# batra-mlp-lab/visdial

Hardware: NVIDIA H100
Metric: QA-rounds/sec mn-att-ques-im-hist+disc train step (higher is better)
Workload: dtype f16 operands + f16 saved state for the option LSTM, tf32 operands elsewhere; fp32 accumulate, fp32 cell state / gradients / optimiser

## Files before the change

visdial_b200/csrc/lstm16.cu:

```cuda
#include <cuda.h>
#include <cuda_fp16.h>
#include <map>
#include <mutex>
#include "../../include/visdial_b200.h"
#include "kernels.cuh"
#include "tc_ptx.cuh"

namespace vd {
namespace tc {

constexpr int BM16 = 128;
constexpr int BK16 = 64;
constexpr int UK16 = 16;
constexpr int BN16 = 128;
constexpr int EW16 = 8;
constexpr int STAGE16 = 32768;

__device__ __forceinline__ float tanh16(float x) { float y; asm("tanh.approx.f32 %0, %1;" : "=f"(y) : "f"(x)); return y; }
__device__ __forceinline__ float sig16(float x) { return fmaf(0.5f, tanh16(0.5f * x), 0.5f); }

__device__ __forceinline__ uint32_t pack2(float a, float b) {
  uint32_t r;
  asm("{\n .reg .f16 lo, hi;\n cvt.rn.satfinite.f16.f32 lo, %1;\n cvt.rn.satfinite.f16.f32 hi, %2;\n mov.b32 %0, {lo, hi};\n}"
      : "=r"(r) : "f"(a), "f"(b));
// ... 10 lines not shown

constexpr int T16_BYTES = 1024, T32_BYTES = 2048;
__device__ __forceinline__ uint8_t* t16_at(uint8_t* base, int row, int unit) {
  return base + row * 64 + (((unit >> 3) ^ ((row >> 1) & 3)) << 4) + (unit & 7) * 2;
}
__device__ __forceinline__ uint8_t* t32_at(uint8_t* base, int row, int unit) {
  return base + row * 128 + (((unit >> 2) ^ (row & 7)) << 4) + (unit & 3) * 4;
}
__device__ __forceinline__ const void* shfl_vptr(const void* p, int src_lane) {
  unsigned long long v = (unsigned long long)p;
  unsigned lo = __shfl_sync(0xffffffffu, (unsigned)v, src_lane), hi = __shfl_sync(0xffffffffu, (unsigned)(v >> 32), src_lane);
  return (const void*)(((unsigned long long)hi << 32) | lo);
}
__device__ __forceinline__ void cp16(void* dst, const void* src) {
  asm volatile("cp.async.cg.shared.global [%0], [%1], 16;" ::"r"(smem_u32(dst)), "l"(src) : "memory");
}
__device__ __forceinline__ void t16_load(uint8_t* base, const void* mine, int lane) {
#pragma unroll
  for (int ps = 0; ps < 2; ++ps) {
    const int row = ps * 8 + (lane >> 2), c = lane & 3;
    const uint8_t* src = (const uint8_t*)shfl_vptr(mine, row);
    uint8_t* dst = base + row * 64 + ((c ^ ((row >> 1) & 3)) << 4);
    if (src) cp16(dst, src + c * 16); else *reinterpret_cast<uint4*>(dst) = make_uint4(0, 0, 0, 0);
  }
}
__device__ __forceinline__ void t32_load(uint8_t* base, const void* mine, int lane) {
#pragma unroll
  for (int ps = 0; ps < 4; ++ps) {
    const int row = ps * 4 + (lane >> 3), c = lane & 7;
    const uint8_t* src = (const uint8_t*)shfl_vptr(mine, row);
    uint8_t* dst = base + row * 128 + ((c ^ (row & 7)) << 4);
    if (src) cp16(dst, src + c * 16); else *reinterpret_cast<float4*>(dst) = make_float4(0.f, 0.f, 0.f, 0.f);
  }
}
__device__ __forceinline__ void cp_wait_all() {
  asm volatile("cp.async.wait_all;" ::: "memory");
  __syncwarp();
}
__device__ __forceinline__ float2 ld_h2(uint8_t* p) { return __half22float2(*reinterpret_cast<const __half2*>(p)); }
__device__ __forceinline__ void st_h2(uint8_t* p, float a, float b) { *reinterpret_cast<uint32_t*>(p) = pack2(a, b); }

struct Lstm16Params {
  int R, H;
  const __half* ptable; const int32_t* tok;
  const float* bias;
  const float* c_prev;
  const int32_t* mask_ids;
  float* h32_out;
  int save_gates;
  const __half* gsave; const float* c_cur; float* dc_carry;
};
struct Lstm16Maps { CUtensorMap g16, c, h16; };

template <int MODE>
struct Cfg16 {
  static constexpr int THREADS = 128 + 32 * EW16;
  static constexpr int STG_PER_WARP = MODE == 0 ? (5 * T16_BYTES + T32_BYTES) : (4 * T16_BYTES + 3 * T32_BYTES);
  static constexpr int STG_BYTES = EW16 * STG_PER_WARP;
  static constexpr int STAGES = (232448 - 1024 - 256 - STG_BYTES) / STAGE16;
  static constexpr int TOTAL = STAGES * STAGE16 + STG_BYTES + 1024 + 256;
};

template <int MODE>
__global__ void __launch_bounds__(Cfg16<MODE>::THREADS, 1)
k_lstm16(const __grid_constant__ CUtensorMap tmA, const __grid_constant__ CUtensorMap tmB,
         const __grid_constant__ Lstm16Maps em, const Lstm16Params p) {
  using C = Cfg16<MODE>;
  constexpr int STAGES = C::STAGES;
  extern __shared__ uint8_t smem_raw[];
  uint8_t* smem = (uint8_t*)(((uintptr_t)smem_raw + 1023) & ~(uintptr_t)1023);
  uint8_t* stg_all = smem + STAGES * STAGE16;
  uint64_t* full = (uint64_t*)(stg_all + C::STG_BYTES);
  uint64_t* empty = full + STAGES;

  const int warp = threadIdx.x >> 5, lane = threadIdx.x & 31;
  const int H = p.H;
  const int num_m = (p.R + BM16 - 1) / BM16;
  const int num_n = MODE == 0 ? H / 32 : H / BN16;
  const int num_tiles = num_m * num_n;
  const int num_kb = (MODE == 0 ? H : 4 * H) / BK16;

  if (threadIdx.x == 0) {
    for (int s = 0; s < STAGES; ++s) { mbar_init(&full[s], 1); mbar_init(&empty[s], 2); }
    asm volatile("fence.mbarrier_init.release.cluster;" ::: "memory");
  }
  __syncthreads();

  if (warp < 4) {
    if (threadIdx.x == 0) {
      int s = 0; uint32_t ph = 0;
      for (int tile = blockIdx.x; tile < num_tiles; tile += gridDim.x) {
        const int m0 = (tile / num_n) * BM16;
        const int nt = tile % num_n;
        for (int kb = 0; kb < num_kb; ++kb) {
          mbar_wait(&empty[s], ph ^ 1);
          uint8_t* sa = smem + s * STAGE16;
          uint8_t* sb = sa + 16384;
          mbar_expect_tx(&full[s], STAGE16);
          tma_load_2d(sa, &tmA, &full[s], kb * BK16, m0);
          if (MODE == 0) {
#pragma unroll
            for (int g = 0; g < 4; ++g) tma_load_2d(sb + g * 4096, &tmB, &full[s], kb * BK16, g * H + nt * 32);
          } else {
            tma_load_2d(sb, &tmB, &full[s], kb * BK16, nt * BN16);
          }
          if (++s == STAGES) { s = 0; ph ^= 1; }
        }
      }
    }
  } else {
    const int cw = warp - 4, wg = cw >> 2;
    uint8_t* stg = stg_all + cw * C::STG_PER_WARP;
    const int fr = lane >> 2, fu = 2 * (lane & 3);
    int s = 0; uint32_t ph = 0;
    auto contract = [&](float (&d)[BN16 / 2]) {
#pragma unroll
      for (int i = 0; i < BN16 / 2; ++i) d[i] = 0.f;
      int prev = -1;
      for (int kb = 0; kb < num_kb; ++kb) {
        mbar_wait(&full[s], ph);
        const uint32_t sa = smem_u32(smem + s * STAGE16);
        const uint64_t adesc = make_desc(sa + wg * 64 * 128, 16, 1024), bdesc = make_desc(sa + 16384, 16, 1024);
        wgmma_fence();
#pragma unroll
        for (int k = 0; k < BK16 / UK16; ++k)
          wgmma_f16_n128(d, adesc + (uint64_t)(k * 2), bdesc + (uint64_t)(k * 2), (kb | k) ? 1u : 0u);
        wgmma_commit();
        wgmma_wait<1>();
        if (prev >= 0 && (threadIdx.x & 127) == 0) mbar_arrive(&empty[prev]);
        prev = s;
        if (++s == STAGES) { s = 0; ph ^= 1; }
      }
      wgmma_wait<0>();
      wgmma_hold(d);
      if (prev >= 0 && (threadIdx.x & 127) == 0) mbar_arrive(&empty[prev]);
    };
    if constexpr (MODE == 0) {
      uint8_t* sG = stg; uint8_t* sH = stg + 4 * T16_BYTES; uint8_t* sC = sH + T16_BYTES;
      for (int tile = blockIdx.x; tile < num_tiles; tile += gridDim.x) {
        const int m0 = (tile / num_n) * BM16;
        const int nt = tile % num_n;
        const int r0 = m0 + wg * 64 + (cw & 3) * 16;
        const int j0 = nt * 32;
        const int64_t row = (int64_t)r0 + (lane & 15);
        const bool row_ok = row < p.R;
        const float keep = (row_ok && p.mask_ids && p.mask_ids[row] == 0) ? 0.f : 1.f;
        const int32_t tk = row_ok ? __ldg(p.tok + row) : 0;
        const __half* prow = tk != 0 ? p.ptable + (int64_t)tk * 4 * H + j0 : nullptr;
        const float* cprow = (row_ok && p.c_prev) ? p.c_prev + row * H + j0 : nullptr;
        if (lane == 0) bulk_wait_read0();
        __syncwarp();
#pragma unroll
        for (int g = 0; g < 4; ++g) t16_load(sG + g * T16_BYTES, prow ? prow + g * H : nullptr, lane);
        t32_load(sC, cprow, lane);
        float d[BN16 / 2];
        contract(d);
        cp_wait_all();
#pragma unroll
        for (int hh = 0; hh < 2; ++hh) {
          const int r = fr + 8 * hh;
          const float kp = __shfl_sync(0xffffffffu, keep, r);
          const int64_t grow = (int64_t)r0 + r;
#pragma unroll
          for (int jj = 0; jj < 4; ++jj) {
            const int u = 8 * jj + fu;
            float a[4][2], cp[2], hn[2];
#pragma unroll
            for (int g = 0; g < 4; ++g) {
              const float2 x = ld_h2(t16_at(sG + g * T16_BYTES, r, u));
              const float2 b = __ldg(reinterpret_cast<const float2*>(p.bias + g * H + j0 + u));
              a[g][0] = d[4 * (jj + 4 * g) + 2 * hh] + (x.x + b.x);
              a[g][1] = d[4 * (jj + 4 * g) + 2 * hh + 1] + (x.y + b.y);
            }
            const float2 c2 = *reinterpret_cast<const float2*>(t32_at(sC, r, u));
            cp[0] = c2.x; cp[1] = c2.y;
#pragma unroll
            for (int e = 0; e < 2; ++e) {
              const float gi = sig16(a[0][e]), gf = sig16(a[1][e]), go = sig16(a[2][e]), gg = tanh16(a[3][e]);
              const float c_ = (gf * cp[e] + gi * gg) * kp;
              a[0][e] = gi * kp; a[1][e] = gf * kp; a[2][e] = go * kp; a[3][e] = gg * kp;
              cp[e] = c_; hn[e] = go * tanh16(c_) * kp;
            }
#pragma unroll
            for (int g = 0; g < 4; ++g) st_h2(t16_at(sG + g * T16_BYTES, r, u), a[g][0], a[g][1]);
            *reinterpret_cast<float2*>(t32_at(sC, r, u)) = make_float2(cp[0], cp[1]);
            st_h2(t16_at(sH, r, u), hn[0], hn[1]);
            if (p.h32_out && grow < p.R)
              *reinterpret_cast<float2*>(p.h32_out + grow * H + j0 + u) = make_float2(hn[0], hn[1]);
          }
        }
        fence_proxy_async_smem();
        __syncwarp();
        if (lane == 0) {
          if (p.save_gates) {
#pragma unroll
            for (int g = 0; g < 4; ++g) tma_store_2d(&em.g16, sG + g * T16_BYTES, g * H + j0, r0);
          }
          tma_store_2d(&em.c, sC, j0, r0);
          tma_store_2d(&em.h16, sH, j0, r0);
          bulk_commit();
        }
        __syncwarp();
      }
    } else {
      uint8_t* sG = stg; uint8_t* sCP = stg + 4 * T16_BYTES; uint8_t* sCC = sCP + T32_BYTES; uint8_t* sDC = sCC + T32_BYTES;
      for (int tile = blockIdx.x; tile < num_tiles; tile += gridDim.x) {
        const int m0 = (tile / num_n) * BM16;
        const int nt = tile % num_n;
        const int r0 = m0 + wg * 64 + (cw & 3) * 16;
        const int64_t row = (int64_t)r0 + (lane & 15);
        const bool row_ok = row < p.R;
        const float keep = (row_ok && p.mask_ids && p.mask_ids[row] == 0) ? 0.f : 1.f;
        const __half* grow = row_ok ? p.gsave + row * 4 * H : nullptr;
        const float* cprow = (row_ok && p.c_prev) ? p.c_prev + row * H : nullptr;
        const float* ccrow = row_ok ? p.c_cur + row * H : nullptr;
        const float* dcrow = row_ok ? p.dc_carry + row * H : nullptr;
        auto fetch = [&](int j) {
          if (lane == 0) bulk_wait_read0();
          __syncwarp();
#pragma unroll
          for (int g = 0; g < 4; ++g) t16_load(sG + g * T16_BYTES, grow ? grow + g * H + j : nullptr, lane);
          t32_load(sCP, cprow ? cprow + j : nullptr, lane);
          t32_load(sCC, ccrow ? ccrow + j : nullptr, lane);
          t32_load(sDC, dcrow ? dcrow + j : nullptr, lane);
        };
        fetch(nt * BN16);
        float d[BN16 / 2];
        contract(d);
#pragma unroll
        for (int grp = 0; grp < BN16 / 32; ++grp) {
          const int j = nt * BN16 + grp * 32;
          if (grp > 0) fetch(j);
          cp_wait_all();
#pragma unroll
          for (int hh = 0; hh < 2; ++hh) {
            const int r = fr + 8 * hh;
            const float keep_r = __shfl_sync(0xffffffffu, keep, r);
#pragma unroll
            for (int jj = 0; jj < 4; ++jj) {
              const int u = 8 * jj + fu;
              float g[4][2], cp[2], cc[2], dc[2], out[4][2], dcn[2];
#pragma unroll
              for (int gg = 0; gg < 4; ++gg) {
                const float2 x = ld_h2(t16_at(sG + gg * T16_BYTES, r, u));
                g[gg][0] = x.x; g[gg][1] = x.y;
              }
              const float2 cp2 = *reinterpret_cast<const float2*>(t32_at(sCP, r, u));
              const float2 cc2 = *reinterpret_cast<const float2*>(t32_at(sCC, r, u));
              const float2 dc2 = *reinterpret_cast<const float2*>(t32_at(sDC, r, u));
              cp[0] = cp2.x; cp[1] = cp2.y; cc[0] = cc2.x; cc[1] = cc2.y; dc[0] = dc2.x; dc[1] = dc2.y;
#pragma unroll
              for (int e = 0; e < 2; ++e) {
                const float dh = d[4 * (4 * grp + jj) + 2 * hh + e];
                const float gi = g[0][e], gf = g[1][e], go = g[2][e], gg_ = g[3][e];
                const float tcv = tanh16(cc[e]);
                const float dd = (dc[e] + dh * go * (1.f - tcv * tcv)) * keep_r;
                const float dhe = dh * keep_r;
                out[0][e] = dd * gg_ * gi * (1.f - gi);
                out[1][e] = dd * cp[e] * gf * (1.f - gf);
                out[2][e] = dhe * tcv * go * (1.f - go);
                out[3][e] = dd * gi * (1.f - gg_ * gg_);
                dcn[e] = dd * gf;
              }
#pragma unroll
              for (int gg = 0; gg < 4; ++gg) st_h2(t16_at(sG + gg * T16_BYTES, r, u), out[gg][0], out[gg][1]);
              *reinterpret_cast<float2*>(t32_at(sDC, r, u)) = make_float2(dcn[0], dcn[1]);
            }
          }
          fence_proxy_async_smem();
          __syncwarp();
          if (lane == 0) {
#pragma unroll
            for (int gg = 0; gg < 4; ++gg) tma_store_2d(&em.g16, sG + gg * T16_BYTES, gg * H + j, r0);
            tma_store_2d(&em.c, sDC, j, r0);
            bulk_commit();
          }
          __syncwarp();
        }
      }
    }
    if (lane == 0) asm volatile("cp.async.bulk.wait_group 0;" ::: "memory");
  }
}

constexpr int A16_KB = 64;
constexpr int A16_BM = 128, A16_BN = 256;
constexpr int A16_THREADS = 384;
constexpr int A16_A_BYTES = (A16_BM / 64) * A16_KB * 128;
constexpr int A16_B_BYTES = (A16_BN / 64) * A16_KB * 128;
constexpr int A16_STAGE = A16_A_BYTES + A16_B_BYTES;
constexpr int A16_STAGES = 4;
constexpr int A16_TOTAL = A16_STAGES * A16_STAGE + 1024 + 256;
constexpr int A16_CHUNKS_PER_CTA = 24;
constexpr int A16_MIN_CHUNK = 32;
struct Atb16Params {
  int M, N, tiles_n, tiles, kbt;
  int chunk, num_chunks;
  float* C; int64_t ldc; const float* inv_scale;
  int* counter;
};

template <bool VEC4>
__global__ void __launch_bounds__(A16_THREADS, 1)
k_atb16(const __grid_constant__ CUtensorMap tmA, const __grid_constant__ CUtensorMap tmB, const Atb16Params p) {
  extern __shared__ uint8_t smem_raw[];
  uint8_t* smem = (uint8_t*)(((uintptr_t)smem_raw + 1023) & ~(uintptr_t)1023);
  uint64_t* full = (uint64_t*)(smem + A16_STAGES * A16_STAGE);
  uint64_t* empty = full + A16_STAGES;
  int* tag = (int*)(empty + A16_STAGES);
  const int warp = threadIdx.x >> 5;

  if (threadIdx.x == 0) {
    for (int s = 0; s < A16_STAGES; ++s) { mbar_init(&full[s], 1); mbar_init(&empty[s], 2); }
    asm volatile("fence.mbarrier_init.release.cluster;" ::: "memory");
  }
  __syncthreads();

  if (warp < 4) {
    if (threadIdx.x == 0) {
      int s = 0; uint32_t ph = 0;
      for (;;) {
        const int c = atomicAdd(p.counter, 1);
        if (c >= p.num_chunks) break;
        const int tile = c % p.tiles, kb0 = (c / p.tiles) * p.chunk, kb1 = min(p.kbt, kb0 + p.chunk);
        const int m0 = (tile / p.tiles_n) * A16_BM, n0 = (tile % p.tiles_n) * A16_BN;
        for (int kb = kb0; kb < kb1; ++kb) {
          const int krow = kb * A16_KB;
          mbar_wait(&empty[s], ph ^ 1);
          uint8_t* sa = smem + s * A16_STAGE;
          uint8_t* sb = sa + A16_A_BYTES;
          if (kb == kb0) tag[s] = c;
          mbar_expect_tx(&full[s], A16_STAGE);
// ... 207 lines not shown
  for (int c0 = threadIdx.x * 8; c0 < ncols; c0 += blockDim.x * 8) {
    float acc[8];
#pragma unroll
    for (int e = 0; e < 8; ++e) acc[e] = 0.f;
    int cur = sorted_tok[p0];
    auto flush = [&](int tok) {
      float* o = out + (int64_t)tok * ncols + c0;
      red_add_v4(o, acc[0] * sc, acc[1] * sc, acc[2] * sc, acc[3] * sc);
      red_add_v4(o + 4, acc[4] * sc, acc[5] * sc, acc[6] * sc, acc[7] * sc);
    };
    for (int64_t p = p0; p < p1; ++p) {
      const int tok = sorted_tok[p];
      if (tok != cur) {
        flush(cur);
#pragma unroll
        for (int e = 0; e < 8; ++e) acc[e] = 0.f;
        cur = tok;
      }
      float v[8];
      unpack8(__ldcs(reinterpret_cast<const uint4*>(X + (int64_t)perm[p] * ldx + c0)), v);
#pragma unroll
      for (int e = 0; e < 8; ++e) acc[e] += v[e];
    }
    flush(cur);
  }
}

static CUtensorMap make_tmap16(const void* base, CUtensorMapDataType dt, int esize, int64_t rows, int64_t cols, int64_t ld,
                               int box_rows, int box_cols, CUtensorMapSwizzle swz) {
  CUtensorMap tm;
  cuuint64_t dims[2] = {(cuuint64_t)cols, (cuuint64_t)rows};
  cuuint64_t strides[1] = {(cuuint64_t)ld * esize};
  cuuint32_t box[2] = {(cuuint32_t)box_cols, (cuuint32_t)box_rows};
  cuuint32_t estr[2] = {1, 1};
  CUresult r = get_encode()(&tm, dt, 2, (void*)base, dims, strides, box, estr, CU_TENSOR_MAP_INTERLEAVE_NONE, swz,
                            CU_TENSOR_MAP_L2_PROMOTION_L2_256B, CU_TENSOR_MAP_FLOAT_OOB_FILL_NONE);
  if (r != CUDA_SUCCESS) {
    char buf[256];
    snprintf(buf, sizeof(buf), "cuTensorMapEncodeTiled (lstm16) failed (%d): base %p rows %lld cols %lld ld %lld box %dx%d", (int)r, base,
             (long long)rows, (long long)cols, (long long)ld, box_rows, box_cols);
    throw CudaError(-3, buf);
  }
  return tm;
}
static CUtensorMap tmap_h(const __half* base, int64_t rows, int64_t cols, int64_t ld, int box_rows, int box_cols,
                          CUtensorMapSwizzle swz) {
  return make_tmap16(base, CU_TENSOR_MAP_DATA_TYPE_FLOAT16, 2, rows, cols, ld, box_rows, box_cols, swz);
}
static CUtensorMap tmap_f(const float* base, int64_t rows, int64_t cols, int64_t ld, int box_rows, int box_cols,
                          CUtensorMapSwizzle swz) {
  return make_tmap16(base, CU_TENSOR_MAP_DATA_TYPE_FLOAT32, 4, rows, cols, ld, box_rows, box_cols, swz);
}

template <int MODE>
static void launch16(LaunchCtx& cx, const CUtensorMap& tA, const CUtensorMap& tB, const Lstm16Maps& em, const Lstm16Params& p,
                     int num_tiles) {
  using C = Cfg16<MODE>;
  static bool attr_set = false;
  if (!attr_set) {
    VD_CUDA_CHECK(cudaFuncSetAttribute(k_lstm16<MODE>, cudaFuncAttributeMaxDynamicSharedMemorySize, C::TOTAL));
    attr_set = true;
  }
  const int pmax = cx.sms();
  int grid = num_tiles;
  if (num_tiles > pmax) { const int rounds = cdiv(num_tiles, pmax); grid = cdiv(num_tiles, rounds); }
  k_lstm16<MODE><<<grid, C::THREADS, C::TOTAL, cx.stream>>>(tA, tB, em, p);
  check_launch(cx, "k_lstm16");
}

}

bool lstm16_shape_ok(int64_t R, int H) { return H % 256 == 0 && H <= 512 && R >= 1024; }

void lstm16_step_fwd(LaunchCtx& cx, int64_t R, int H, const __half* h_prev16, const __half* Wh16, const __half* ptable16,
                     const int32_t* tok, const float* bias, const float* c_prev, const int32_t* mask_ids, __half* gates16,
                     float* c_out, __half* h16_out, float* h32_out) {
  using namespace tc;
  VD_REQUIRE(lstm16_shape_ok(R, H), VD_E_STATE, "lstm16_step_fwd: shape");
  Lstm16Params p = {};
  p.R = (int)R; p.H = H; p.ptable = ptable16; p.tok = tok; p.bias = bias; p.c_prev = c_prev; p.mask_ids = mask_ids;
  p.h32_out = h32_out; p.save_gates = gates16 != nullptr;
  CUtensorMap tA = tmap_h(h_prev16, R, H, H, BM16, BK16, CU_TENSOR_MAP_SWIZZLE_128B);
  CUtensorMap tB = tmap_h(Wh16, 4 * (int64_t)H, H, H, 32, BK16, CU_TENSOR_MAP_SWIZZLE_128B);
  Lstm16Maps em;
  em.g16 = gates16 ? tmap_h(gates16, R, 4 * (int64_t)H, 4 * (int64_t)H, 16, 32, CU_TENSOR_MAP_SWIZZLE_64B)
                   : tmap_h(h16_out, R, H, H, 16, 32, CU_TENSOR_MAP_SWIZZLE_64B);
  em.c = tmap_f(c_out, R, H, H, 16, 32, CU_TENSOR_MAP_SWIZZLE_128B);
  em.h16 = tmap_h(h16_out, R, H, H, 16, 32, CU_TENSOR_MAP_SWIZZLE_64B);
  launch16<0>(cx, tA, tB, em, p, cdiv(R, BM16) * (H / 32));
}

void lstm16_step_bwd(LaunchCtx& cx, int64_t R, int H, const __half* da_next16, const __half* Whb16, const __half* gates16,
                     const float* c_prev, const float* c_cur, float* dc_carry, const int32_t* mask_ids, __half* da16) {
  using namespace tc;
  VD_REQUIRE(lstm16_shape_ok(R, H), VD_E_STATE, "lstm16_step_bwd: shape");
  Lstm16Params p = {};
  p.R = (int)R; p.H = H; p.gsave = gates16; p.c_prev = c_prev; p.c_cur = c_cur; p.dc_carry = dc_carry; p.mask_ids = mask_ids;
  CUtensorMap tA = tmap_h(da_next16, R, 4 * (int64_t)H, 4 * (int64_t)H, BM16, BK16, CU_TENSOR_MAP_SWIZZLE_128B);
  CUtensorMap tB = tmap_h(Whb16, H, 4 * (int64_t)H, 4 * (int64_t)H, 128, BK16, CU_TENSOR_MAP_SWIZZLE_128B);
  Lstm16Maps em;
  em.g16 = tmap_h(da16, R, 4 * (int64_t)H, 4 * (int64_t)H, 16, 32, CU_TENSOR_MAP_SWIZZLE_64B);
  em.c = tmap_f(dc_carry, R, H, H, 16, 32, CU_TENSOR_MAP_SWIZZLE_128B);
  em.h16 = em.c;
  launch16<1>(cx, tA, tB, em, p, cdiv(R, BM16) * (H / BN16));
}

void lstm16_first_step(LaunchCtx& cx, int64_t R, int H, const __half* ptable16, const int32_t* tok, const float* bias,
                       const float* c_prev, const int32_t* mask_ids, __half* gates16, float* c_out, __half* h16_out, float* h32_out) {
  const int64_t n = R * (H / 8);
  tc::k_lstm16_first<<<(unsigned)((n + 255) / 256), 256, 0, cx.stream>>>(ptable16, tok, bias, c_prev, mask_ids, gates16, c_out,
                                                                          h16_out, h32_out, R, H);
  check_launch(cx, "k_lstm16_first");
}

void lstm16_bwd_last(LaunchCtx& cx, int64_t R, int H, const __half* gates16, const float* c_prev, const float* c_cur,
                     const float* dh_last, const float* scale, const int32_t* mask_ids, float* dc_carry, __half* da16) {
  const int64_t n = R * (H / 8);
  tc::k_lstm16_bwd_last<<<(unsigned)((n + 255) / 256), 256, 0, cx.stream>>>(gates16, c_prev, c_cur, dh_last, scale, mask_ids,
                                                                             dc_carry, da16, R, H);
  check_launch(cx, "k_lstm16_bwd_last");
}

void cvt_f32_to_f16(LaunchCtx& cx, __half* dst, int64_t ldd, const float* src, int64_t lds, int64_t rows, int cols) {
  VD_REQUIRE(cols % 4 == 0 && lds % 4 == 0 && ldd % 4 == 0, VD_E_STATE, "cvt_f32_to_f16: alignment");
  const int64_t n = rows * (cols / 4);
  if (n == 0) return;
  tc::k_cvt16<<<(unsigned)((n + 255) / 256), 256, 0, cx.stream>>>(dst, ldd, src, lds, rows, cols);
  check_launch(cx, "k_cvt16");
}

void pick_grad_scale(LaunchCtx& cx, const float* x, int64_t n, uint32_t* bits, float* scale2) {
  VD_REQUIRE(n % 4 == 0, VD_E_STATE, "pick_grad_scale: n % 4");
  VD_CUDA_CHECK(cudaMemsetAsync(bits, 0, sizeof(uint32_t), cx.stream));
  const int blocks = (int)std::min<int64_t>((n / 4 + 255) / 256, 4 * cx.sm_count);
  tc::k_amax<<<blocks, 256, 0, cx.stream>>>(x, n / 4, bits);
  check_launch(cx, "k_amax");
  tc::k_pick_scale<<<1, 1, 0, cx.stream>>>(bits, scale2);
  check_launch(cx, "k_pick_scale");
}

void segsum_rows16(LaunchCtx& cx, const __half* X, int64_t ldx, const int32_t* perm, const int32_t* sorted_tok, int64_t n,
                   float* out, int ncols, const float* inv_scale) {
  VD_REQUIRE(ncols % 8 == 0 && ldx % 8 == 0, VD_E_STATE, "segsum_rows16: alignment");
  if (n == 0) return;
  tc::k_segsum16<<<(unsigned)((n + tc::SEG16_ROWS - 1) / tc::SEG16_ROWS), 256, 0, cx.stream>>>(X, ldx, perm, sorted_tok, n, out, ncols,
                                                                                               inv_scale);
  check_launch(cx, "k_segsum16");
}

static int* atb16_counter(cudaStream_t stream) {
  static std::mutex mu;
  static std::map<std::pair<int, cudaStream_t>, int*> counters;
  int dev = 0;
  VD_CUDA_CHECK(cudaGetDevice(&dev));
  std::lock_guard<std::mutex> lock(mu);
  int*& c = counters[{dev, stream}];
  if (!c) {
// ... 35 lines not shown
```

visdial_b200/csrc/tc_ptx.cuh:

```cuda
#pragma once
#include <cuda.h>
#include <stdint.h>

namespace vd {
namespace tc {

__device__ __forceinline__ uint32_t smem_u32(const void* p) { return (uint32_t)__cvta_generic_to_shared(p); }

__device__ __forceinline__ void mbar_init(uint64_t* bar, uint32_t count) {
  asm volatile("mbarrier.init.shared::cta.b64 [%0], %1;" ::"r"(smem_u32(bar)), "r"(count));
}
__device__ __forceinline__ void mbar_expect_tx(uint64_t* bar, uint32_t bytes) {
  asm volatile("mbarrier.arrive.expect_tx.shared::cta.b64 _, [%0], %1;" ::"r"(smem_u32(bar)), "r"(bytes) : "memory");
}
__device__ __forceinline__ void mbar_arrive(uint64_t* bar) {
  asm volatile("mbarrier.arrive.shared::cta.b64 _, [%0];" ::"r"(smem_u32(bar)) : "memory");
}
__device__ __forceinline__ void mbar_wait(uint64_t* bar, uint32_t parity) {
  uint32_t done = 0, spins = 0;
  uint32_t addr = smem_u32(bar);
  while (!done) {
    asm volatile(
        "{\n .reg .pred p;\n mbarrier.try_wait.parity.shared::cta.b64 p, [%1], %2;\n selp.u32 %0, 1, 0, p;\n}"
        : "=r"(done) : "r"(addr), "r"(parity) : "memory");
    if (!done && ++spins > (1u << 24)) __trap();
  }
}
__device__ __forceinline__ void tma_load_2d(void* smem_dst, const CUtensorMap* tm, uint64_t* bar, int c0, int c1) {
  asm volatile(
      "cp.async.bulk.tensor.2d.shared::cluster.global.mbarrier::complete_tx::bytes [%0], [%1, {%3, %4}], [%2];"
      ::"r"(smem_u32(smem_dst)), "l"(tm), "r"(smem_u32(bar)), "r"(c0), "r"(c1) : "memory");
}
__device__ __forceinline__ void wgmma_fence() { asm volatile("wgmma.fence.sync.aligned;" ::: "memory"); }
__device__ __forceinline__ void wgmma_commit() { asm volatile("wgmma.commit_group.sync.aligned;" ::: "memory"); }
template <int N> __device__ __forceinline__ void wgmma_wait() { asm volatile("wgmma.wait_group.sync.aligned %0;" ::"n"(N) : "memory"); }
template <int NR> __device__ __forceinline__ void wgmma_hold(float (&d)[NR]) {
#pragma unroll
  for (int i = 0; i < NR; ++i) asm volatile("" : "+f"(d[i])::"memory");
}
__device__ __forceinline__ void bar_named(int id, int threads) { asm volatile("bar.sync %0, %1;" ::"r"(id), "r"(threads) : "memory"); }

__device__ __forceinline__ uint64_t make_desc(uint32_t saddr, uint32_t lbo_bytes, uint32_t sbo_bytes) {
  uint64_t d = 0;
  d |= (uint64_t)((saddr & 0x3FFFF) >> 4);
  d |= (uint64_t)((lbo_bytes >> 4) & 0x3FFF) << 16;
  d |= (uint64_t)((sbo_bytes >> 4) & 0x3FFF) << 32;
  d |= (uint64_t)1 << 62;
  return d;
}

__device__ __forceinline__ void wgmma_tf32_n32(float (&d)[16], uint64_t a, uint64_t b, uint32_t acc) {
  asm volatile(
      "{\n .reg .pred p;\n setp.ne.b32 p, %18, 0;\n"
      "wgmma.mma_async.sync.aligned.m64n32k8.f32.tf32.tf32 {%0, %1, %2, %3, %4, %5, %6, %7, %8, %9, %10, %11, %12, %13, %14, %15}, %16, %17, p, 1, 1;\n}\n"
      : "+f"(d[0]), "+f"(d[1]), "+f"(d[2]), "+f"(d[3]), "+f"(d[4]), "+f"(d[5]), "+f"(d[6]), "+f"(d[7]), "+f"(d[8]), "+f"(d[9]), "+f"(d[10]), "+f"(d[11]), "+f"(d[12]), "+f"(d[13]), "+f"(d[14]), "+f"(d[15])
      : "l"(a), "l"(b), "r"(acc));
}

__device__ __forceinline__ void wgmma_tf32_n64(float (&d)[32], uint64_t a, uint64_t b, uint32_t acc) {
  asm volatile(
      "{\n .reg .pred p;\n setp.ne.b32 p, %34, 0;\n"
      "wgmma.mma_async.sync.aligned.m64n64k8.f32.tf32.tf32 {%0, %1, %2, %3, %4, %5, %6, %7, %8, %9, %10, %11, %12, %13, %14, %15, %16, %17, %18, %19, %20, %21, %22, %23, %24, %25, %26, %27, %28, %29, %30, %31}, %32, %33, p, 1, 1;\n}\n"
      : "+f"(d[0]), "+f"(d[1]), "+f"(d[2]), "+f"(d[3]), "+f"(d[4]), "+f"(d[5]), "+f"(d[6]), "+f"(d[7]), "+f"(d[8]), "+f"(d[9]), "+f"(d[10]), "+f"(d[11]), "+f"(d[12]), "+f"(d[13]), "+f"(d[14]), "+f"(d[15]), "+f"(d[16]), "+f"(d[17]), "+f"(d[18]), "+f"(d[19]), "+f"(d[20]), "+f"(d[21]), "+f"(d[22]), "+f"(d[23]), "+f"(d[24]), "+f"(d[25]), "+f"(d[26]), "+f"(d[27]), "+f"(d[28]), "+f"(d[29]), "+f"(d[30]), "+f"(d[31])
      : "l"(a), "l"(b), "r"(acc));
}

__device__ __forceinline__ void wgmma_tf32_n128(float (&d)[64], uint64_t a, uint64_t b, uint32_t acc) {
  asm volatile(
      "{\n .reg .pred p;\n setp.ne.b32 p, %66, 0;\n"
      "wgmma.mma_async.sync.aligned.m64n128k8.f32.tf32.tf32 {%0, %1, %2, %3, %4, %5, %6, %7, %8, %9, %10, %11, %12, %13, %14, %15, %16, %17, %18, %19, %20, %21, %22, %23, %24, %25, %26, %27, %28, %29, %30, %31, %32, %33, %34, %35, %36, %37, %38, %39, %40, %41, %42, %43, %44, %45, %46, %47, %48, %49, %50, %51, %52, %53, %54, %55, %56, %57, %58, %59, %60, %61, %62, %63}, %64, %65, p, 1, 1;\n}\n"
      : "+f"(d[0]), "+f"(d[1]), "+f"(d[2]), "+f"(d[3]), "+f"(d[4]), "+f"(d[5]), "+f"(d[6]), "+f"(d[7]), "+f"(d[8]), "+f"(d[9]), "+f"(d[10]), "+f"(d[11]), "+f"(d[12]), "+f"(d[13]), "+f"(d[14]), "+f"(d[15]), "+f"(d[16]), "+f"(d[17]), "+f"(d[18]), "+f"(d[19]), "+f"(d[20]), "+f"(d[21]), "+f"(d[22]), "+f"(d[23]), "+f"(d[24]), "+f"(d[25]), "+f"(d[26]), "+f"(d[27]), "+f"(d[28]), "+f"(d[29]), "+f"(d[30]), "+f"(d[31]), "+f"(d[32]), "+f"(d[33]), "+f"(d[34]), "+f"(d[35]), "+f"(d[36]), "+f"(d[37]), "+f"(d[38]), "+f"(d[39]), "+f"(d[40]), "+f"(d[41]), "+f"(d[42]), "+f"(d[43]), "+f"(d[44]), "+f"(d[45]), "+f"(d[46]), "+f"(d[47]), "+f"(d[48]), "+f"(d[49]), "+f"(d[50]), "+f"(d[51]), "+f"(d[52]), "+f"(d[53]), "+f"(d[54]), "+f"(d[55]), "+f"(d[56]), "+f"(d[57]), "+f"(d[58]), "+f"(d[59]), "+f"(d[60]), "+f"(d[61]), "+f"(d[62]), "+f"(d[63])
      : "l"(a), "l"(b), "r"(acc));
}

__device__ __forceinline__ void wgmma_f16_n32(float (&d)[16], uint64_t a, uint64_t b, uint32_t acc) {
  asm volatile(
      "{\n .reg .pred p;\n setp.ne.b32 p, %18, 0;\n"
      "wgmma.mma_async.sync.aligned.m64n32k16.f32.f16.f16 {%0, %1, %2, %3, %4, %5, %6, %7, %8, %9, %10, %11, %12, %13, %14, %15}, %16, %17, p, 1, 1, 0, 0;\n}\n"
      : "+f"(d[0]), "+f"(d[1]), "+f"(d[2]), "+f"(d[3]), "+f"(d[4]), "+f"(d[5]), "+f"(d[6]), "+f"(d[7]), "+f"(d[8]), "+f"(d[9]), "+f"(d[10]), "+f"(d[11]), "+f"(d[12]), "+f"(d[13]), "+f"(d[14]), "+f"(d[15])
      : "l"(a), "l"(b), "r"(acc));
}

__device__ __forceinline__ void wgmma_f16_n128(float (&d)[64], uint64_t a, uint64_t b, uint32_t acc) {
  asm volatile(
      "{\n .reg .pred p;\n setp.ne.b32 p, %66, 0;\n"
      "wgmma.mma_async.sync.aligned.m64n128k16.f32.f16.f16 {%0, %1, %2, %3, %4, %5, %6, %7, %8, %9, %10, %11, %12, %13, %14, %15, %16, %17, %18, %19, %20, %21, %22, %23, %24, %25, %26, %27, %28, %29, %30, %31, %32, %33, %34, %35, %36, %37, %38, %39, %40, %41, %42, %43, %44, %45, %46, %47, %48, %49, %50, %51, %52, %53, %54, %55, %56, %57, %58, %59, %60, %61, %62, %63}, %64, %65, p, 1, 1, 0, 0;\n}\n"
      : "+f"(d[0]), "+f"(d[1]), "+f"(d[2]), "+f"(d[3]), "+f"(d[4]), "+f"(d[5]), "+f"(d[6]), "+f"(d[7]), "+f"(d[8]), "+f"(d[9]), "+f"(d[10]), "+f"(d[11]), "+f"(d[12]), "+f"(d[13]), "+f"(d[14]), "+f"(d[15]), "+f"(d[16]), "+f"(d[17]), "+f"(d[18]), "+f"(d[19]), "+f"(d[20]), "+f"(d[21]), "+f"(d[22]), "+f"(d[23]), "+f"(d[24]), "+f"(d[25]), "+f"(d[26]), "+f"(d[27]), "+f"(d[28]), "+f"(d[29]), "+f"(d[30]), "+f"(d[31]), "+f"(d[32]), "+f"(d[33]), "+f"(d[34]), "+f"(d[35]), "+f"(d[36]), "+f"(d[37]), "+f"(d[38]), "+f"(d[39]), "+f"(d[40]), "+f"(d[41]), "+f"(d[42]), "+f"(d[43]), "+f"(d[44]), "+f"(d[45]), "+f"(d[46]), "+f"(d[47]), "+f"(d[48]), "+f"(d[49]), "+f"(d[50]), "+f"(d[51]), "+f"(d[52]), "+f"(d[53]), "+f"(d[54]), "+f"(d[55]), "+f"(d[56]), "+f"(d[57]), "+f"(d[58]), "+f"(d[59]), "+f"(d[60]), "+f"(d[61]), "+f"(d[62]), "+f"(d[63])
      : "l"(a), "l"(b), "r"(acc));
}

__device__ __forceinline__ void wgmma_f16_n256_mn(float (&d)[128], uint64_t a, uint64_t b, uint32_t acc) {
  asm volatile(
      "{\n .reg .pred p;\n setp.ne.b32 p, %130, 0;\n"
// ... 51 lines not shown
```

Before: 16080.

## Keep the recurrent weight slice resident in shared memory for forward LSTM16 step

The forward option-LSTM step kernel is rewritten so that each CTA owns one 32-column gate slice of Wh and loads the whole slice into shared memory once. It then streams only 64-row A tiles through a small ring across several row blocks, so weights are no longer re-fetched for every tile. The two consumer warpgroups are serialized with named-barrier tokens so they share the single A ring in order. This adds a shared-memory capacity limit (H up to 512), more complex synchronisation, and a grid of slices times balanced workers.

Result: faster. 16570, median of 6 (+3.1%).

```diff
diff --git a/visdial_b200/csrc/lstm16.cu b/visdial_b200/csrc/lstm16.cu
--- a/visdial_b200/csrc/lstm16.cu
+++ b/visdial_b200/csrc/lstm16.cu
@@ -86,10 +86,27 @@
 };
 struct Lstm16Maps { CUtensorMap g16, c, h16; };
 
-template <int MODE>
-struct Cfg16 {
+template <int MODE> struct Cfg16;
+
+template <>
+struct Cfg16<0> {
   static constexpr int THREADS = 128 + 32 * EW16;
-  static constexpr int STG_PER_WARP = MODE == 0 ? (5 * T16_BYTES + T32_BYTES) : (4 * T16_BYTES + 3 * T32_BYTES);
+  static constexpr int KB_MAX = 512 / BK16;
+  static constexpr int SLICE_KB = 4 * 32 * BK16 * 2;
+  static constexpr int RES_BYTES = KB_MAX * SLICE_KB;
+  static constexpr int A_STAGE = 64 * BK16 * 2;
+  static constexpr int A_STAGES = 5;
+  static constexpr int STG_PER_WARP = 5 * T16_BYTES + T32_BYTES;
+  static constexpr int STG_BYTES = EW16 * STG_PER_WARP;
+  static constexpr int BAR_BYTES = 8 * (KB_MAX + 2 * A_STAGES);
+  static constexpr int TOTAL = RES_BYTES + A_STAGES * A_STAGE + STG_BYTES + BAR_BYTES + 1024;
+  static_assert(TOTAL <= 232448, "k_lstm16<0>: shared memory");
+};
+
+template <>
+struct Cfg16<1> {
+  static constexpr int THREADS = 128 + 32 * EW16;
+  static constexpr int STG_PER_WARP = 4 * T16_BYTES + 3 * T32_BYTES;
   static constexpr int STG_BYTES = EW16 * STG_PER_WARP;
   static constexpr int STAGES = (232448 - 1024 - 256 - STG_BYTES) / STAGE16;
   static constexpr int TOTAL = STAGES * STAGE16 + STG_BYTES + 1024 + 256;
@@ -99,6 +116,7 @@
 __global__ void __launch_bounds__(Cfg16<MODE>::THREADS, 1)
 k_lstm16(const __grid_constant__ CUtensorMap tmA, const __grid_constant__ CUtensorMap tmB,
          const __grid_constant__ Lstm16Maps em, const Lstm16Params p) {
+  static_assert(MODE == 1, "the forward step is the k_lstm16<0> specialisation below");
   using C = Cfg16<MODE>;
   constexpr int STAGES = C::STAGES;
   extern __shared__ uint8_t smem_raw[];
@@ -110,9 +128,9 @@
   const int warp = threadIdx.x >> 5, lane = threadIdx.x & 31;
   const int H = p.H;
   const int num_m = (p.R + BM16 - 1) / BM16;
-  const int num_n = MODE == 0 ? H / 32 : H / BN16;
+  const int num_n = H / BN16;
   const int num_tiles = num_m * num_n;
-  const int num_kb = (MODE == 0 ? H : 4 * H) / BK16;
+  const int num_kb = 4 * H / BK16;
 
   if (threadIdx.x == 0) {
     for (int s = 0; s < STAGES; ++s) { mbar_init(&full[s], 1); mbar_init(&empty[s], 2); }
@@ -132,12 +150,7 @@
           uint8_t* sb = sa + 16384;
           mbar_expect_tx(&full[s], STAGE16);
           tma_load_2d(sa, &tmA, &full[s], kb * BK16, m0);
-          if (MODE == 0) {
-#pragma unroll
-            for (int g = 0; g < 4; ++g) tma_load_2d(sb + g * 4096, &tmB, &full[s], kb * BK16, g * H + nt * 32);
-          } else {
-            tma_load_2d(sb, &tmB, &full[s], kb * BK16, nt * BN16);
-          }
+          tma_load_2d(sb, &tmB, &full[s], kb * BK16, nt * BN16);
           if (++s == STAGES) { s = 0; ph ^= 1; }
         }
       }
@@ -169,149 +182,241 @@
       wgmma_hold(d);
       if (prev >= 0 && (threadIdx.x & 127) == 0) mbar_arrive(&empty[prev]);
     };
-    if constexpr (MODE == 0) {
-      uint8_t* sG = stg; uint8_t* sH = stg + 4 * T16_BYTES; uint8_t* sC = sH + T16_BYTES;
-      for (int tile = blockIdx.x; tile < num_tiles; tile += gridDim.x) {
-        const int m0 = (tile / num_n) * BM16;
-        const int nt = tile % num_n;
-        const int r0 = m0 + wg * 64 + (cw & 3) * 16;
-        const int j0 = nt * 32;
-        const int64_t row = (int64_t)r0 + (lane & 15);
-        const bool row_ok = row < p.R;
-        const float keep = (row_ok && p.mask_ids && p.mask_ids[row] == 0) ? 0.f : 1.f;
-        const int32_t tk = row_ok ? __ldg(p.tok + row) : 0;
-        const __half* prow = tk != 0 ? p.ptable + (int64_t)tk * 4 * H + j0 : nullptr;
-        const float* cprow = (row_ok && p.c_prev) ? p.c_prev + row * H + j0 : nullptr;
+    uint8_t* sG = stg; uint8_t* sCP = stg + 4 * T16_BYTES; uint8_t* sCC = sCP + T32_BYTES; uint8_t* sDC = sCC + T32_BYTES;
+    for (int tile = blockIdx.x; tile < num_tiles; tile += gridDim.x) {
+      const int m0 = (tile / num_n) * BM16;
+      const int nt = tile % num_n;
+      const int r0 = m0 + wg * 64 + (cw & 3) * 16;
+      const int64_t row = (int64_t)r0 + (lane & 15);
+      const bool row_ok = row < p.R;
+      const float keep = (row_ok && p.mask_ids && p.mask_ids[row] == 0) ? 0.f : 1.f;
+      const __half* grow = row_ok ? p.gsave + row * 4 * H : nullptr;
+      const float* cprow = (row_ok && p.c_prev) ? p.c_prev + row * H : nullptr;
+      const float* ccrow = row_ok ? p.c_cur + row * H : nullptr;
+      const float* dcrow = row_ok ? p.dc_carry + row * H : nullptr;
+      auto fetch = [&](int j) {
         if (lane == 0) bulk_wait_read0();
         __syncwarp();
 #pragma unroll
-        for (int g = 0; g < 4; ++g) t16_load(sG + g * T16_BYTES, prow ? prow + g * H : nullptr, lane);
-        t32_load(sC, cprow, lane);
-        float d[BN16 / 2];
-        contract(d);
+        for (int g = 0; g < 4; ++g) t16_load(sG + g * T16_BYTES, grow ? grow + g * H + j : nullptr, lane);
+        t32_load(sCP, cprow ? cprow + j : nullptr, lane);
+        t32_load(sCC, ccrow ? ccrow + j : nullptr, lane);
+        t32_load(sDC, dcrow ? dcrow + j : nullptr, lane);
+      };
+      fetch(nt * BN16);
+      float d[BN16 / 2];
+      contract(d);
+#pragma unroll
+      for (int grp = 0; grp < BN16 / 32; ++grp) {
+        const int j = nt * BN16 + grp * 32;
+        if (grp > 0) fetch(j);
         cp_wait_all();
 #pragma unroll
         for (int hh = 0; hh < 2; ++hh) {
           const int r = fr + 8 * hh;
-          const float kp = __shfl_sync(0xffffffffu, keep, r);
-          const int64_t grow = (int64_t)r0 + r;
+          const float keep_r = __shfl_sync(0xffffffffu, keep, r);
 #pragma unroll
           for (int jj = 0; jj < 4; ++jj) {
             const int u = 8 * jj + fu;
-            float a[4][2], cp[2], hn[2];
-#pragma unroll
-            for (int g = 0; g < 4; ++g) {
-              const float2 x = ld_h2(t16_at(sG + g * T16_BYTES, r, u));
-              const float2 b = __ldg(reinterpret_cast<const float2*>(p.bias + g * H + j0 + u));
-              a[g][0] = d[4 * (jj + 4 * g) + 2 * hh] + (x.x + b.x);
-              a[g][1] = d[4 * (jj + 4 * g) + 2 * hh + 1] + (x.y + b.y);
+            float g[4][2], cp[2], cc[2], dc[2], out[4][2], dcn[2];
+#pragma unroll
+            for (int gg = 0; gg < 4; ++gg) {
+              const float2 x = ld_h2(t16_at(sG + gg * T16_BYTES, r, u));
+              g[gg][0] = x.x; g[gg][1] = x.y;
             }
-            const float2 c2 = *reinterpret_cast<const float2*>(t32_at(sC, r, u));
-            cp[0] = c2.x; cp[1] = c2.y;
+            const float2 cp2 = *reinterpret_cast<const float2*>(t32_at(sCP, r, u));
+            const float2 cc2 = *reinterpret_cast<const float2*>(t32_at(sCC, r, u));
+            const float2 dc2 = *reinterpret_cast<const float2*>(t32_at(sDC, r, u));
+            cp[0] = cp2.x; cp[1] = cp2.y; cc[0] = cc2.x; cc[1] = cc2.y; dc[0] = dc2.x; dc[1] = dc2.y;
 #pragma unroll
             for (int e = 0; e < 2; ++e) {
-              const float gi = sig16(a[0][e]), gf = sig16(a[1][e]), go = sig16(a[2][e]), gg = tanh16(a[3][e]);
-              const float c_ = (gf * cp[e] + gi * gg) * kp;
-              a[0][e] = gi * kp; a[1][e] = gf * kp; a[2][e] = go * kp; a[3][e] = gg * kp;
-              cp[e] = c_; hn[e] = go * tanh16(c_) * kp;
+              const float dh = d[4 * (4 * grp + jj) + 2 * hh + e];
+              const float gi = g[0][e], gf = g[1][e], go = g[2][e], gg_ = g[3][e];
+              const float tcv = tanh16(cc[e]);
+              const float dd = (dc[e] + dh * go * (1.f - tcv * tcv)) * keep_r;
+              const float dhe = dh * keep_r;
+              out[0][e] = dd * gg_ * gi * (1.f - gi);
+              out[1][e] = dd * cp[e] * gf * (1.f - gf);
+              out[2][e] = dhe * tcv * go * (1.f - go);
+              out[3][e] = dd * gi * (1.f - gg_ * gg_);
+              dcn[e] = dd * gf;
             }
 #pragma unroll
-            for (int g = 0; g < 4; ++g) st_h2(t16_at(sG + g * T16_BYTES, r, u), a[g][0], a[g][1]);
-            *reinterpret_cast<float2*>(t32_at(sC, r, u)) = make_float2(cp[0], cp[1]);
-            st_h2(t16_at(sH, r, u), hn[0], hn[1]);
-            if (p.h32_out && grow < p.R)
-              *reinterpret_cast<float2*>(p.h32_out + grow * H + j0 + u) = make_float2(hn[0], hn[1]);
+            for (int gg = 0; gg < 4; ++gg) st_h2(t16_at(sG + gg * T16_BYTES, r, u), out[gg][0], out[gg][1]);
+            *reinterpret_cast<float2*>(t32_at(sDC, r, u)) = make_float2(dcn[0], dcn[1]);
           }
         }
         fence_proxy_async_smem();
         __syncwarp();
         if (lane == 0) {
-          if (p.save_gates) {
-#pragma unroll
-            for (int g = 0; g < 4; ++g) tma_store_2d(&em.g16, sG + g * T16_BYTES, g * H + j0, r0);
-          }
-          tma_store_2d(&em.c, sC, j0, r0);
-          tma_store_2d(&em.h16, sH, j0, r0);
+#pragma unroll
+          for (int gg = 0; gg < 4; ++gg) tma_store_2d(&em.g16, sG + gg * T16_BYTES, gg * H + j, r0);
+          tma_store_2d(&em.c, sDC, j, r0);
           bulk_commit();
         }
         __syncwarp();
       }
-    } else {
-      uint8_t* sG = stg; uint8_t* sCP = stg + 4 * T16_BYTES; uint8_t* sCC = sCP + T32_BYTES; uint8_t* sDC = sCC + T32_BYTES;
-      for (int tile = blockIdx.x; tile < num_tiles; tile += gridDim.x) {
-        const int m0 = (tile / num_n) * BM16;
-        const int nt = tile % num_n;
-        const int r0 = m0 + wg * 64 + (cw & 3) * 16;
-        const int64_t row = (int64_t)r0 + (lane & 15);
-        const bool row_ok = row < p.R;
-        const float keep = (row_ok && p.mask_ids && p.mask_ids[row] == 0) ? 0.f : 1.f;
-        const __half* grow = row_ok ? p.gsave + row * 4 * H : nullptr;
-        const float* cprow = (row_ok && p.c_prev) ? p.c_prev + row * H : nullptr;
-        const float* ccrow = row_ok ? p.c_cur + row * H : nullptr;
-        const float* dcrow = row_ok ? p.dc_carry + row * H : nullptr;
-        auto fetch = [&](int j) {
-          if (lane == 0) bulk_wait_read0();
-          __syncwarp();
-#pragma unroll
-          for (int g = 0; g < 4; ++g) t16_load(sG + g * T16_BYTES, grow ? grow + g * H + j : nullptr, lane);
-          t32_load(sCP, cprow ? cprow + j : nullptr, lane);
-          t32_load(sCC, ccrow ? ccrow + j : nullptr, lane);
-          t32_load(sDC, dcrow ? dcrow + j : nullptr, lane);
-        };
-        fetch(nt * BN16);
-        float d[BN16 / 2];
-        contract(d);
-#pragma unroll
-        for (int grp = 0; grp < BN16 / 32; ++grp) {
-          const int j = nt * BN16 + grp * 32;
-          if (grp > 0) fetch(j);
-          cp_wait_all();
-#pragma unroll
-          for (int hh = 0; hh < 2; ++hh) {
-            const int r = fr + 8 * hh;
-            const float keep_r = __shfl_sync(0xffffffffu, keep, r);
-#pragma unroll
-            for (int jj = 0; jj < 4; ++jj) {
-              const int u = 8 * jj + fu;
-              float g[4][2], cp[2], cc[2], dc[2], out[4][2], dcn[2];
-#pragma unroll
-              for (int gg = 0; gg < 4; ++gg) {
-                const float2 x = ld_h2(t16_at(sG + gg * T16_BYTES, r, u));
-                g[gg][0] = x.x; g[gg][1] = x.y;
-              }
-              const float2 cp2 = *reinterpret_cast<const float2*>(t32_at(sCP, r, u));
-              const float2 cc2 = *reinterpret_cast<const float2*>(t32_at(sCC, r, u));
-              const float2 dc2 = *reinterpret_cast<const float2*>(t32_at(sDC, r, u));
-              cp[0] = cp2.x; cp[1] = cp2.y; cc[0] = cc2.x; cc[1] = cc2.y; dc[0] = dc2.x; dc[1] = dc2.y;
-#pragma unroll
-              for (int e = 0; e < 2; ++e) {
-                const float dh = d[4 * (4 * grp + jj) + 2 * hh + e];
-                const float gi = g[0][e], gf = g[1][e], go = g[2][e], gg_ = g[3][e];
-                const float tcv = tanh16(cc[e]);
-                const float dd = (dc[e] + dh * go * (1.f - tcv * tcv)) * keep_r;
-                const float dhe = dh * keep_r;
-                out[0][e] = dd * gg_ * gi * (1.f - gi);
-                out[1][e] = dd * cp[e] * gf * (1.f - gf);
-                out[2][e] = dhe * tcv * go * (1.f - go);
-                out[3][e] = dd * gi * (1.f - gg_ * gg_);
-                dcn[e] = dd * gf;
-              }
-#pragma unroll
-              for (int gg = 0; gg < 4; ++gg) st_h2(t16_at(sG + gg * T16_BYTES, r, u), out[gg][0], out[gg][1]);
-              *reinterpret_cast<float2*>(t32_at(sDC, r, u)) = make_float2(dcn[0], dcn[1]);
-            }
+    }
+    if (lane == 0) asm volatile("cp.async.bulk.wait_group 0;" ::: "memory");
+  }
+}
+
+template <>
+__global__ void __launch_bounds__(Cfg16<0>::THREADS, 1)
+k_lstm16<0>(const __grid_constant__ CUtensorMap tmA, const __grid_constant__ CUtensorMap tmB,
+            const __grid_constant__ Lstm16Maps em, const Lstm16Params p) {
+  using C = Cfg16<0>;
+  constexpr int AS = C::A_STAGES;
+  constexpr int TOKEN_WG1 = 1, TOKEN_WG2 = 2;
+  extern __shared__ uint8_t smem_raw[];
+  uint8_t* smem = (uint8_t*)(((uintptr_t)smem_raw + 1023) & ~(uintptr_t)1023);
+  uint8_t* slice = smem;
+  uint8_t* ring = slice + C::RES_BYTES;
+  uint8_t* stg_all = ring + AS * C::A_STAGE;
+  uint64_t* wfull = (uint64_t*)(stg_all + C::STG_BYTES);
+  uint64_t* full = wfull + C::KB_MAX;
+  uint64_t* empty = full + AS;
+
+  const int warp = threadIdx.x >> 5, lane = threadIdx.x & 31;
+  const int H = p.H;
+  const int num_m = (p.R + BM16 - 1) / BM16;
+  const int num_n = H / 32;
+  const int num_kb = H / BK16;
+  const int nt = blockIdx.x % num_n, per = gridDim.x / num_n;
+  const int mb0 = blockIdx.x / num_n;
+
+  if (threadIdx.x == 0) {
+    for (int kb = 0; kb < num_kb; ++kb) mbar_init(&wfull[kb], 1);
+    for (int s = 0; s < AS; ++s) { mbar_init(&full[s], 1); mbar_init(&empty[s], 1); }
+    asm volatile("fence.mbarrier_init.release.cluster;" ::: "memory");
+  }
+  __syncthreads();
+
+  if (warp < 4) {
+    if (threadIdx.x == 0 && mb0 < num_m) {
+      for (int kb = 0; kb < num_kb; ++kb) {
+        uint8_t* sb = slice + kb * C::SLICE_KB;
+        mbar_expect_tx(&wfull[kb], C::SLICE_KB);
+#pragma unroll
+        for (int g = 0; g < 4; ++g) tma_load_2d(sb + g * 4096, &tmB, &wfull[kb], kb * BK16, g * H + nt * 32);
+      }
+      int s = 0; uint32_t ph = 0;
+      for (int mb = mb0; mb < num_m; mb += per) {
+        for (int w = 0; w < 2; ++w) {
+          for (int kb = 0; kb < num_kb; ++kb) {
+            mbar_wait(&empty[s], ph ^ 1);
+            mbar_expect_tx(&full[s], C::A_STAGE);
+            tma_load_2d(ring + s * C::A_STAGE, &tmA, &full[s], kb * BK16, mb * BM16 + w * 64);
+            if (++s == AS) { s = 0; ph ^= 1; }
           }
-          fence_proxy_async_smem();
-          __syncwarp();
-          if (lane == 0) {
-#pragma unroll
-            for (int gg = 0; gg < 4; ++gg) tma_store_2d(&em.g16, sG + gg * T16_BYTES, gg * H + j, r0);
-            tma_store_2d(&em.c, sDC, j, r0);
-            bulk_commit();
+        }
+      }
+    }
+  } else {
+    const int cw = warp - 4, wg = cw >> 2;
+    uint8_t* stg = stg_all + cw * C::STG_PER_WARP;
+    const int fr = lane >> 2, fu = 2 * (lane & 3);
+    int s = 0; uint32_t ph = 0;
+    auto skip = [&](int n) {
+      for (s += n; s >= AS; s -= AS) ph ^= 1;
+    };
+    skip(wg * num_kb);
+    auto contract = [&](float (&d)[BN16 / 2], bool first) {
+#pragma unroll
+      for (int i = 0; i < BN16 / 2; ++i) d[i] = 0.f;
+      int prev = -1;
+      for (int kb = 0; kb < num_kb; ++kb) {
+        if (first) mbar_wait(&wfull[kb], 0);
+        mbar_wait(&full[s], ph);
+        const uint64_t adesc = make_desc(smem_u32(ring + s * C::A_STAGE), 16, 1024),
+                       bdesc = make_desc(smem_u32(slice + kb * C::SLICE_KB), 16, 1024);
+        wgmma_fence();
+#pragma unroll
+        for (int k = 0; k < BK16 / UK16; ++k)
+          wgmma_f16_n128(d, adesc + (uint64_t)(k * 2), bdesc + (uint64_t)(k * 2), (kb | k) ? 1u : 0u);
+        wgmma_commit();
+        wgmma_wait<1>();
+        if (prev >= 0 && (threadIdx.x & 127) == 0) mbar_arrive(&empty[prev]);
+        prev = s;
+        if (++s == AS) { s = 0; ph ^= 1; }
+      }
+      wgmma_wait<0>();
+      wgmma_hold(d);
+      if (prev >= 0 && (threadIdx.x & 127) == 0) mbar_arrive(&empty[prev]);
+      skip(num_kb);
+    };
+    uint8_t* sG = stg; uint8_t* sH = stg + 4 * T16_BYTES; uint8_t* sC = sH + T16_BYTES;
+    for (int mb = mb0; mb < num_m; mb += per) {
+      int j0 = nt * 32;
+      asm volatile("" : "+r"(j0));
+      const int r0 = mb * BM16 + wg * 64 + (cw & 3) * 16;
+      const int64_t row = (int64_t)r0 + (lane & 15);
+      const bool row_ok = row < p.R;
+      const float keep = (row_ok && p.mask_ids && p.mask_ids[row] == 0) ? 0.f : 1.f;
+      const int32_t tk = row_ok ? __ldg(p.tok + row) : 0;
+      const __half* prow = tk != 0 ? p.ptable + (int64_t)tk * 4 * H + j0 : nullptr;
+      const float* cprow = (row_ok && p.c_prev) ? p.c_prev + row * H + j0 : nullptr;
+      if (lane == 0) bulk_wait_read0();
+      __syncwarp();
+#pragma unroll
+      for (int g = 0; g < 4; ++g) t16_load(sG + g * T16_BYTES, prow ? prow + g * H : nullptr, lane);
+      t32_load(sC, cprow, lane);
+      const bool first = mb == mb0;
+      if (wg == 0) {
+        if (!first) bar_named(TOKEN_WG1, 256);
+      } else {
+        bar_named(TOKEN_WG2, 256);
+      }
+      float d[BN16 / 2];
+      contract(d, first);
+      if (wg == 0) bar_arrive_named(TOKEN_WG2, 256);
+      else if (mb + per < num_m) bar_arrive_named(TOKEN_WG1, 256);
+      cp_wait_all();
+#pragma unroll
+      for (int hh = 0; hh < 2; ++hh) {
+        const int r = fr + 8 * hh;
+        const float kp = __shfl_sync(0xffffffffu, keep, r);
+        const int64_t grow = (int64_t)r0 + r;
+#pragma unroll
+        for (int jj = 0; jj < 4; ++jj) {
+          const int u = 8 * jj + fu;
+          float a[4][2], cp[2], hn[2];
+#pragma unroll
+          for (int g = 0; g < 4; ++g) {
+            const float2 x = ld_h2(t16_at(sG + g * T16_BYTES, r, u));
+            const float2 b = __ldg(reinterpret_cast<const float2*>(p.bias + g * H + j0 + u));
+            a[g][0] = d[4 * (jj + 4 * g) + 2 * hh] + (x.x + b.x);
+            a[g][1] = d[4 * (jj + 4 * g) + 2 * hh + 1] + (x.y + b.y);
           }
-          __syncwarp();
+          const float2 c2 = *reinterpret_cast<const float2*>(t32_at(sC, r, u));
+          cp[0] = c2.x; cp[1] = c2.y;
+#pragma unroll
+          for (int e2 = 0; e2 < 2; ++e2) {
+            const float gi = sig16(a[0][e2]), gf = sig16(a[1][e2]), go = sig16(a[2][e2]), gg = tanh16(a[3][e2]);
+            const float c_ = (gf * cp[e2] + gi * gg) * kp;
+            a[0][e2] = gi * kp; a[1][e2] = gf * kp; a[2][e2] = go * kp; a[3][e2] = gg * kp;
+            cp[e2] = c_; hn[e2] = go * tanh16(c_) * kp;
+          }
+#pragma unroll
+          for (int g = 0; g < 4; ++g) st_h2(t16_at(sG + g * T16_BYTES, r, u), a[g][0], a[g][1]);
+          *reinterpret_cast<float2*>(t32_at(sC, r, u)) = make_float2(cp[0], cp[1]);
+          st_h2(t16_at(sH, r, u), hn[0], hn[1]);
+          if (p.h32_out && grow < p.R)
+            *reinterpret_cast<float2*>(p.h32_out + grow * H + j0 + u) = make_float2(hn[0], hn[1]);
         }
       }
+      fence_proxy_async_smem();
+      __syncwarp();
+      if (lane == 0) {
+        if (p.save_gates) {
+#pragma unroll
+          for (int g = 0; g < 4; ++g) tma_store_2d(&em.g16, sG + g * T16_BYTES, g * H + j0, r0);
+        }
+        tma_store_2d(&em.c, sC, j0, r0);
+        tma_store_2d(&em.h16, sH, j0, r0);
+        bulk_commit();
+      }
+      __syncwarp();
     }
     if (lane == 0) asm volatile("cp.async.bulk.wait_group 0;" ::: "memory");
   }
@@ -625,18 +730,17 @@
   return make_tmap16(base, CU_TENSOR_MAP_DATA_TYPE_FLOAT32, 4, rows, cols, ld, box_rows, box_cols, swz);
 }
 
+static int balanced_workers(int n, int pmax) { return n <= pmax ? n : cdiv(n, cdiv(n, pmax)); }
+
 template <int MODE>
 static void launch16(LaunchCtx& cx, const CUtensorMap& tA, const CUtensorMap& tB, const Lstm16Maps& em, const Lstm16Params& p,
-                     int num_tiles) {
+                     int grid) {
   using C = Cfg16<MODE>;
   static bool attr_set = false;
   if (!attr_set) {
     VD_CUDA_CHECK(cudaFuncSetAttribute(k_lstm16<MODE>, cudaFuncAttributeMaxDynamicSharedMemorySize, C::TOTAL));
     attr_set = true;
   }
-  const int pmax = cx.sms();
-  int grid = num_tiles;
-  if (num_tiles > pmax) { const int rounds = cdiv(num_tiles, pmax); grid = cdiv(num_tiles, rounds); }
   k_lstm16<MODE><<<grid, C::THREADS, C::TOTAL, cx.stream>>>(tA, tB, em, p);
   check_launch(cx, "k_lstm16");
 }
@@ -653,14 +757,15 @@
   Lstm16Params p = {};
   p.R = (int)R; p.H = H; p.ptable = ptable16; p.tok = tok; p.bias = bias; p.c_prev = c_prev; p.mask_ids = mask_ids;
   p.h32_out = h32_out; p.save_gates = gates16 != nullptr;
-  CUtensorMap tA = tmap_h(h_prev16, R, H, H, BM16, BK16, CU_TENSOR_MAP_SWIZZLE_128B);
+  CUtensorMap tA = tmap_h(h_prev16, R, H, H, 64, BK16, CU_TENSOR_MAP_SWIZZLE_128B);
   CUtensorMap tB = tmap_h(Wh16, 4 * (int64_t)H, H, H, 32, BK16, CU_TENSOR_MAP_SWIZZLE_128B);
   Lstm16Maps em;
   em.g16 = gates16 ? tmap_h(gates16, R, 4 * (int64_t)H, 4 * (int64_t)H, 16, 32, CU_TENSOR_MAP_SWIZZLE_64B)
                    : tmap_h(h16_out, R, H, H, 16, 32, CU_TENSOR_MAP_SWIZZLE_64B);
   em.c = tmap_f(c_out, R, H, H, 16, 32, CU_TENSOR_MAP_SWIZZLE_128B);
   em.h16 = tmap_h(h16_out, R, H, H, 16, 32, CU_TENSOR_MAP_SWIZZLE_64B);
-  launch16<0>(cx, tA, tB, em, p, cdiv(R, BM16) * (H / 32));
+  const int slices = H / 32;
+  launch16<0>(cx, tA, tB, em, p, slices * balanced_workers(cdiv(R, BM16), std::max(1, cx.sms() / slices)));
 }
 
 void lstm16_step_bwd(LaunchCtx& cx, int64_t R, int H, const __half* da_next16, const __half* Whb16, const __half* gates16,
@@ -675,7 +780,7 @@
   em.g16 = tmap_h(da16, R, 4 * (int64_t)H, 4 * (int64_t)H, 16, 32, CU_TENSOR_MAP_SWIZZLE_64B);
   em.c = tmap_f(dc_carry, R, H, H, 16, 32, CU_TENSOR_MAP_SWIZZLE_128B);
   em.h16 = em.c;
-  launch16<1>(cx, tA, tB, em, p, cdiv(R, BM16) * (H / BN16));
+  launch16<1>(cx, tA, tB, em, p, balanced_workers(cdiv(R, BM16) * (H / BN16), cx.sms()));
 }
 
 void lstm16_first_step(LaunchCtx& cx, int64_t R, int H, const __half* ptable16, const int32_t* tok, const float* bias,
diff --git a/visdial_b200/csrc/tc_ptx.cuh b/visdial_b200/csrc/tc_ptx.cuh
--- a/visdial_b200/csrc/tc_ptx.cuh
+++ b/visdial_b200/csrc/tc_ptx.cuh
@@ -39,6 +39,7 @@
   for (int i = 0; i < NR; ++i) asm volatile("" : "+f"(d[i])::"memory");
 }
 __device__ __forceinline__ void bar_named(int id, int threads) { asm volatile("bar.sync %0, %1;" ::"r"(id), "r"(threads) : "memory"); }
+__device__ __forceinline__ void bar_arrive_named(int id, int threads) { asm volatile("bar.arrive %0, %1;" ::"r"(id), "r"(threads) : "memory"); }
 
 __device__ __forceinline__ uint64_t make_desc(uint32_t saddr, uint32_t lbo_bytes, uint32_t sbo_bytes) {
   uint64_t d = 0;
```
